# xqtr/PySpecSDR

Measured on AMD Instinct MI355X. Metric: IQ MSamples/sec end-to-end (FFT+dB+FM demod), higher is better.
Workload: dtype complex64 IQ / f64 FFT + dB + post-process + FIR + IIR / dB rows stored as f32 / int16 PCM

## Files before the change

pyspecsdr_amd/csrc/pss_api.cpp:

```cpp
#include <hip/hip_runtime.h>

#include <cstdlib>
#include <cstring>
#include <string>
#include <vector>

#include "pss_ctx.h"

static std::string g_create_err;

int pss_fail(pss_ctx *ctx, int code, const std::string &msg)
{
    if (ctx) ctx->err = msg;
    else g_create_err = msg;
    return code;
}

int pss_hip_check(pss_ctx *ctx, hipError_t e, const char *what)
{
    if (e == hipSuccess) return PSS_OK;
    return pss_fail(ctx, PSS_E_HIP, std::string(what) + ": " + hipGetErrorString(e));
}

int pss_ensure_buffer(pss_ctx *ctx, void **buf, size_t *cap, size_t bytes, const char *what)
{
    if (bytes <= *cap) return PSS_OK;
    if (*buf) {
        hipStreamSynchronize(ctx->stream);
        if (ctx->stream2) hipStreamSynchronize(ctx->stream2);
        hipFree(*buf);
        *buf = nullptr;
        *cap = 0;
    }
    hipError_t e = hipMalloc(buf, bytes);
    if (e != hipSuccess) return pss_fail(ctx, PSS_E_NOMEM, std::string(what) + " hipMalloc: " + hipGetErrorString(e));
    *cap = bytes;
    return PSS_OK;
}

int pss_ensure_scratch(pss_ctx *ctx, size_t bytes)
{
    return pss_ensure_buffer(ctx, &ctx->scratch, &ctx->scratch_bytes, bytes, "scratch");
}

void pss_time_begin(pss_ctx *ctx)
{
    if (ctx->timing && ctx->tdepth++ == 0 && ctx->tfilter.empty()) hipEventRecord(ctx->ev0, ctx->stream);
}
void pss_kernel_begin(pss_ctx *ctx, const char *name)
{
    if (!ctx->timing) return;
    ctx->kskip = !ctx->tfilter.empty() && ctx->tfilter != name;
    if (ctx->kskip) return;
    if (ctx->kused == (int)ctx->krecs.size()) {
        pss_ctx::KRec r{name, nullptr, nullptr};
        hipEventCreate(&r.e0);
        hipEventCreate(&r.e1);
        ctx->krecs.push_back(r);
    }
    ctx->krecs[ctx->kused].name = name;
    hipEventRecord(ctx->krecs[ctx->kused].e0, PSS_STREAM(ctx));
}
void pss_kernel_end(pss_ctx *ctx)
{
    if (!ctx->timing || ctx->kskip) return;
    hipEventRecord(ctx->krecs[ctx->kused].e1, PSS_STREAM(ctx));
    ctx->kused++;
}
void pss_time_end(pss_ctx *ctx)
{
    if (ctx->timing && --ctx->tdepth == 0) {
        if (ctx->tfilter.empty()) hipEventRecord(ctx->ev1, ctx->stream);
        ctx->last_ms = 0.0f;
    }
}

extern "C" int pss_device_count(void)
{
    int n = 0;
    if (hipGetDeviceCount(&n) != hipSuccess) return 0;
    return n;
}

extern "C" int pss_create(int device, pss_ctx **out)
{
    if (!out) return PSS_E_ARG;
    *out = nullptr;
    int n = 0;
    hipError_t e = hipGetDeviceCount(&n);
    if (e != hipSuccess || n <= 0)
        return pss_fail(nullptr, PSS_E_HIP, std::string("no HIP device available (libpss has no CPU fallback): ") +
                                                (e != hipSuccess ? hipGetErrorString(e) : "device count is 0"));
    if (device < 0 || device >= n) return pss_fail(nullptr, PSS_E_ARG, "device index out of range");
    int prev = -1;
    hipGetDevice(&prev);
    e = hipSetDevice(device);
    if (e != hipSuccess) return pss_fail(nullptr, PSS_E_HIP, std::string("hipSetDevice: ") + hipGetErrorString(e));
    struct Restore {
        int prev, dev;
        ~Restore() { if (prev >= 0 && prev != dev) hipSetDevice(prev); }
    } restore{prev, device};
    pss_ctx *ctx = new pss_ctx();
    ctx->device = device;
    { int cus = 0; if (hipDeviceGetAttribute(&cus, hipDeviceAttributeMultiprocessorCount, device) == hipSuccess) ctx->n_cus = cus; }
    { const char *e = getenv("PSS_NO_FUSED"); ctx->no_fused = e && e[0] == '1'; }
    e = hipStreamCreateWithFlags(&ctx->stream, hipStreamNonBlocking);
    if (e == hipSuccess) ctx->own_stream = true;
    if (e == hipSuccess) e = hipEventCreate(&ctx->ev0);
    if (e == hipSuccess) e = hipEventCreate(&ctx->ev1);
    if (e == hipSuccess) e = hipStreamCreateWithFlags(&ctx->stream2, hipStreamNonBlocking);
    if (e == hipSuccess) e = hipEventCreateWithFlags(&ctx->ev_fork, hipEventDisableTiming);
    if (e == hipSuccess) e = hipEventCreateWithFlags(&ctx->ev_join, hipEventDisableTiming);
    if (e != hipSuccess) {
        const std::string msg = std::string("context stream / event creation: ") + hipGetErrorString(e);
        if (ctx->ev0) hipEventDestroy(ctx->ev0);
        if (ctx->ev1) hipEventDestroy(ctx->ev1);
        if (ctx->ev_fork) hipEventDestroy(ctx->ev_fork);
        if (ctx->ev_join) hipEventDestroy(ctx->ev_join);
        if (ctx->stream2) hipStreamDestroy(ctx->stream2);
        if (ctx->own_stream) hipStreamDestroy(ctx->stream);
        delete ctx;
        return pss_fail(nullptr, PSS_E_HIP, msg);
    }
    *out = ctx;
    return PSS_OK;
}

extern "C" void pss_destroy(pss_ctx *ctx)
{
    if (!ctx) return;
    PssDevGuard guard(ctx->device);
    hipStreamSynchronize(ctx->stream);
    if (ctx->comm) pss_comm_free(ctx);
    for (auto &kv : ctx->tw) hipFree(kv.second);
    for (auto &kv : ctx->tw_pf) hipFree(kv.second);
    for (auto &kv : ctx->win) hipFree(kv.second);
    for (auto &kv : ctx->bs) { hipFree(kv.second.d_chirp); hipFree(kv.second.d_B); hipFree(kv.second.d_win); }
    for (auto &kv : ctx->plans) {
        hipFree(kv.second.d_leaf_off); hipFree(kv.second.d_leaf_len); hipFree(kv.second.d_node_l);
        hipFree(kv.second.d_node_r); hipFree(kv.second.d_level_start); hipFree(kv.second.d_roots);
    }
    for (auto &kv : ctx->nfm) if (kv.second.d_rev) hipFree(kv.second.d_rev);
    if (ctx->scratch) hipFree(ctx->scratch);
    if (ctx->scratch_fft) hipFree(ctx->scratch_fft);
    if (ctx->scratch_hil) hipFree(ctx->scratch_hil);
    if (ctx->scratch_iqc) hipFree(ctx->scratch_iqc);
    if (ctx->d_hann) hipFree(ctx->d_hann);
    if (ctx->d_hann_short) hipFree(ctx->d_hann_short);
    if (ctx->st_up) hipStreamDestroy(ctx->st_up);
    if (ctx->st_dn) hipStreamDestroy(ctx->st_dn);
    for (auto &e : ctx->st_ev) if (e) hipEventDestroy(e);
    for (auto &b : ctx->st_buf) if (b) hipFree(b);
    if (ctx->scratch_scan) hipFree(ctx->scratch_scan);
    if (ctx->scratch_pk) hipFree(ctx->scratch_pk);
    if (ctx->scratch_win) hipFree(ctx->scratch_win);
    if (ctx->scratch_db64) hipFree(ctx->scratch_db64);
    if (ctx->scratch_post) hipFree(ctx->scratch_post);
    if (ctx->prog) hipFree(ctx->prog);
    if (ctx->stage) hipFree(ctx->stage);
    for (auto &b : ctx->sq_buf) if (b) hipFree(b);
    if (ctx->sq_pin) hipHostFree(ctx->sq_pin);
    hipEventDestroy(ctx->ev0);
    hipEventDestroy(ctx->ev1);
    hipStreamSynchronize(ctx->stream2);
    hipStreamDestroy(ctx->stream2);
    hipEventDestroy(ctx->ev_fork);
    hipEventDestroy(ctx->ev_join);
    if (ctx->ev_in) hipEventDestroy(ctx->ev_in);
    if (ctx->ev_out) hipEventDestroy(ctx->ev_out);
    for (auto &k : ctx->krecs) { hipEventDestroy(k.e0); hipEventDestroy(k.e1); }
    if (ctx->own_stream) hipStreamDestroy(ctx->stream);
    delete ctx;
}

extern "C" int pss_set_stream(pss_ctx *ctx, void *hip_stream)
{
    if (!ctx) return PSS_E_ARG;
    PSS_GUARD(ctx);
    hipStreamSynchronize(ctx->stream);
    if (ctx->own_stream) hipStreamDestroy(ctx->stream);
    ctx->stream = reinterpret_cast<hipStream_t>(hip_stream);
    ctx->own_stream = false;
    return PSS_OK;
}

extern "C" int pss_order_after(pss_ctx *ctx, void *hip_stream)
{
    if (!ctx) return PSS_E_ARG;
    PSS_GUARD(ctx);
    hipStream_t s = reinterpret_cast<hipStream_t>(hip_stream);
    if (s == ctx->stream) return PSS_OK;
    if (!ctx->ev_in) PSS_HIP(ctx, hipEventCreateWithFlags(&ctx->ev_in, hipEventDisableTiming));
    PSS_HIP(ctx, hipEventRecord(ctx->ev_in, s));
    PSS_HIP(ctx, hipStreamWaitEvent(ctx->stream, ctx->ev_in, 0));
    return PSS_OK;
}

extern "C" int pss_order_before(pss_ctx *ctx, void *hip_stream)
{
    if (!ctx) return PSS_E_ARG;
    PSS_GUARD(ctx);
    hipStream_t s = reinterpret_cast<hipStream_t>(hip_stream);
    if (s == ctx->stream) return PSS_OK;
    if (!ctx->ev_out) PSS_HIP(ctx, hipEventCreateWithFlags(&ctx->ev_out, hipEventDisableTiming));
    PSS_HIP(ctx, hipEventRecord(ctx->ev_out, ctx->stream));
    PSS_HIP(ctx, hipStreamWaitEvent(s, ctx->ev_out, 0));
    return PSS_OK;
}

extern "C" void *pss_get_stream(pss_ctx *ctx) { return ctx ? reinterpret_cast<void *>(ctx->stream) : nullptr; }

extern "C" int pss_set_option(pss_ctx *ctx, const char *key, int value)
{
    if (!ctx || !key) return PSS_E_ARG;
    if (!strcmp(key, "nfm_fused")) { ctx->no_fused = (value == 0); return PSS_OK; }
    if (!strcmp(key, "wfm_fused")) { ctx->no_wfm_fused = (value == 0); return PSS_OK; }
    if (!strcmp(key, "small_batch")) { ctx->no_small_batch = (value == 0); return PSS_OK; }
    if (!strcmp(key, "small_batch_max")) { ctx->small_batch_max = value; return PSS_OK; }
    if (!strcmp(key, "wfm_small_batch_max")) { ctx->wfm_small_batch_max = value; return PSS_OK; }
    if (!strcmp(key, "fuse_post")) { ctx->fuse_post = value != 0; return PSS_OK; }
    if (!strcmp(key, "ssb_rfft")) { ctx->ssb_rfft = value != 0; return PSS_OK; }
    if (!strcmp(key, "ssb_hilbert")) { ctx->ssb_hilbert = value != 0; return PSS_OK; }
    if (!strcmp(key, "hilbert_exact")) { ctx->hilbert_exact = value != 0; return PSS_OK; }
    if (!strcmp(key, "scan_exact")) { ctx->scan_exact = value != 0; return PSS_OK; }
    if (!strcmp(key, "db_exact")) { ctx->db_exact = value != 0; return PSS_OK; }
    if (!strcmp(key, "f64_plain")) { ctx->f64_plain = value != 0; return PSS_OK; }
    if (!strcmp(key, "wfm_corr_copy")) { ctx->wfm_corr_copy = value != 0; return PSS_OK; }
    return pss_fail(ctx, PSS_E_ARG, std::string("unknown option: ") + key);
}

extern "C" int pss_sync(pss_ctx *ctx)
{
    if (!ctx) return PSS_E_ARG;
    PSS_GUARD(ctx);
    return pss_hip_check(ctx, hipStreamSynchronize(ctx->stream), "hipStreamSynchronize");
}

extern "C" const char *pss_last_error(pss_ctx *ctx) { return ctx ? ctx->err.c_str() : g_create_err.c_str(); }

extern "C" int pss_enable_timing(pss_ctx *ctx, int on)
{
    if (!ctx) return PSS_E_ARG;
    PSS_GUARD(ctx);
    ctx->timing = on != 0;
    ctx->tdepth = 0;
    ctx->kused = 0;
    ctx->last_ms = -1.0f;
    return PSS_OK;
}

extern "C" int pss_timing_filter(pss_ctx *ctx, const char *kernel)
{
    if (!ctx) return PSS_E_ARG;
    PSS_GUARD(ctx);
    ctx->tfilter = kernel ? kernel : "";
    ctx->kused = 0;
    ctx->last_ms = -1.0f;
    return PSS_OK;
}

extern "C" float pss_last_kernel_ms(pss_ctx *ctx)
{
    if (!ctx || !ctx->timing || ctx->last_ms < 0.0f || !ctx->tfilter.empty()) return -1.0f;
    PSS_GUARD(ctx);
    if (hipEventSynchronize(ctx->ev1) != hipSuccess) return -1.0f;
    float ms = -1.0f;
    if (hipEventElapsedTime(&ms, ctx->ev0, ctx->ev1) != hipSuccess) return -1.0f;
    return ms;
}

extern "C" int pss_kernel_times(pss_ctx *ctx, char *buf, int buf_len)
{
    if (!ctx || !buf || buf_len < 1) return PSS_E_ARG;
    PSS_GUARD(ctx);
    std::string out;
    if (ctx->timing && ctx->last_ms >= 0.0f) {
        if (ctx->tfilter.empty()) hipEventSynchronize(ctx->ev1);
        else hipStreamSynchronize(ctx->stream);
        for (int i = 0; i < ctx->kused; i++) {
            float ms = 0.0f;
            if (hipEventElapsedTime(&ms, ctx->krecs[i].e0, ctx->krecs[i].e1) != hipSuccess) continue;
            out += ctx->krecs[i].name;
            out += "=" + std::to_string(ms) + ";";
        }
    }
    ctx->kused = 0;
    if ((int)out.size() + 1 > buf_len) return pss_fail(ctx, PSS_E_ARG, "buffer too small");
    memcpy(buf, out.c_str(), out.size() + 1);
    return PSS_OK;
}

namespace {
size_t up256(size_t x) { return (x + 255) & ~(size_t)255; }
}

extern "C" int pss_h_compute_fft(pss_ctx *ctx, const float *h_iq, int n, double *h_db)
{
    if (!ctx) return PSS_E_ARG;
    PSS_GUARD(ctx);
    if (!h_iq || !h_db || n < 1) return pss_fail(ctx, PSS_E_ARG, "bad arguments");
    const size_t o_db = up256(sizeof(float) * 2 * n);
    int r = pss_ensure_buffer(ctx, &ctx->stage, &ctx->stage_bytes, o_db + up256(sizeof(float) * n), "staging");
    if (r) return r;
    char *base = reinterpret_cast<char *>(ctx->stage);
    PSS_HIP(ctx, hipMemcpyAsync(base, h_iq, sizeof(float) * 2 * n, hipMemcpyHostToDevice, ctx->stream));
    r = pss_spectrum_db(ctx, reinterpret_cast<const float *>(base), 1, n, reinterpret_cast<float *>(base + o_db));
    if (r) return r;
    std::vector<float> tmp(n);
    PSS_HIP(ctx, hipMemcpyAsync(tmp.data(), base + o_db, sizeof(float) * n, hipMemcpyDeviceToHost, ctx->stream));
    PSS_HIP(ctx, hipStreamSynchronize(ctx->stream));
    for (int i = 0; i < n; i++) h_db[i] = (double)tmp[i];
// ... 523 lines not shown
```

pyspecsdr_amd/csrc/pss_ctx.h:

```cpp
#pragma once
#include <hip/hip_runtime.h>

#include <array>
#include <functional>
#include <map>
#include <string>
#include <vector>

#include "../../include/pss.h"

struct PssNfmFilt {
    double taps[65];
    double sos[24];
    double zi[8];
    double *d_rev = nullptr;
};

struct PssWfmFilt {
    double lp[18], pilot[30], lmr[30];
    double alpha;
};

struct PssPairwisePlan {
    int n_leaves = 0, n_nodes = 0, n_levels = 0, n_roots = 0;
    int wave_tree = 0;
    int *d_leaf_off = nullptr, *d_leaf_len = nullptr, *d_node_l = nullptr, *d_node_r = nullptr, *d_level_start = nullptr;
    int *d_roots = nullptr;
};

struct pss_ctx {
    int device = 0;
    hipStream_t stream = nullptr;
    bool own_stream = false;
    hipStream_t stream2 = nullptr;
    hipStream_t cur = nullptr;
    hipEvent_t ev_fork = nullptr, ev_join = nullptr;
    hipEvent_t ev_in = nullptr, ev_out = nullptr;
    int n_cus = 0;
    bool iq_c128 = false;
    int fuse_post = 1;
    double target_rate = 22050.0;
    bool wfm_correct = false;
    const float *wfm_scal = nullptr;
    bool wfm_corr_copy = false;
    float *power_out = nullptr;
    bool fork_after_fwd = false;
    bool did_fork = false;
    bool defer_bwd = false;
    std::function<int()> pending_bwd;
    std::string err;
    std::map<int, double2 *> tw;
    std::map<int, double *> win;
    std::map<int, double2 *> tw_pf;
    struct Bluestein { double2 *d_chirp; double2 *d_B; double *d_win; int M; };
    std::map<int, Bluestein> bs;
    std::map<double, PssNfmFilt> nfm;
    std::map<double, std::array<double, 65>> ssb;
    std::map<double, PssWfmFilt> wfm;
    std::map<int, PssPairwisePlan> plans;
    void *scratch = nullptr;
    size_t scratch_bytes = 0;
    void *scratch_iqc = nullptr;
    void *scratch_scan = nullptr;
    size_t scratch_scan_bytes = 0;
    void *scratch_pk = nullptr;
    size_t scratch_pk_bytes = 0;
    void *prog = nullptr;
    unsigned prog_epoch = 0;
    void *scratch_post = nullptr;
    size_t scratch_post_bytes = 0;
    void *scratch_db64 = nullptr;
    size_t scratch_db64_bytes = 0;
    void *scratch_win = nullptr;
    size_t scratch_win_bytes = 0;
    float *d_hann = nullptr;
    float hann_sum = 0.0f;
    hipStream_t st_up = nullptr, st_dn = nullptr;
    hipEvent_t st_ev[6] = {nullptr, nullptr, nullptr, nullptr, nullptr, nullptr};
    void *st_buf[18] = {};
    size_t st_cap[18] = {};
    float *d_hann_short = nullptr;
    float hann_short_sum = 0.0f;
    int hann_short_n = 0;
    size_t scratch_iqc_bytes = 0;
    void *scratch_fft = nullptr;
    size_t scratch_fft_bytes = 0;
    void *scratch_hil = nullptr;
    size_t scratch_hil_bytes = 0;
    void *stage = nullptr;
    size_t stage_bytes = 0;
    bool no_wfm_fused = false;
    long small_batch_max = 8192;
    long wfm_small_batch_max = 6000;
    bool hilbert_exact = false;
    bool ssb_rfft = true;
    bool ssb_hilbert = true;
    bool db_exact = false;
    bool f64_plain = false;
    bool scan_exact = true;
    bool no_small_batch = false;
    bool no_fused = false;
    void *comm = nullptr;
    int comm_rank = 0, comm_n = 1;
    void *sq_buf[3] = {};
    size_t sq_cap[3] = {};
    void *sq_pin = nullptr;
    bool timing = false;
    std::string tfilter;
    bool kskip = false;
    int tdepth = 0;
    hipEvent_t ev0 = nullptr, ev1 = nullptr;
    float last_ms = -1.0f;
    struct KRec { const char *name; hipEvent_t e0, e1; };
    std::vector<KRec> krecs;
    int kused = 0;
};

struct PssDevGuard {
    int prev = -1;
    bool switched = false;
    explicit PssDevGuard(int dev)
    {
        if (hipGetDevice(&prev) == hipSuccess && prev != dev) switched = hipSetDevice(dev) == hipSuccess;
    }
    ~PssDevGuard()
    {
        if (switched) hipSetDevice(prev);
    }
    PssDevGuard(const PssDevGuard &) = delete;
    PssDevGuard &operator=(const PssDevGuard &) = delete;
};
#define PSS_GUARD(ctx) PssDevGuard _pss_dev_guard((ctx)->device)

template <class T>
struct PssScoped {
    T &ref;
    T keep;
    PssScoped(T &r, T v) : ref(r), keep(r) { r = v; }
    ~PssScoped() { ref = keep; }
    PssScoped(const PssScoped &) = delete;
    PssScoped &operator=(const PssScoped &) = delete;
};
using PssFlagScope = PssScoped<bool>;
using PssStreamScope = PssScoped<hipStream_t>;

int pss_fail(pss_ctx *ctx, int code, const std::string &msg);
int pss_hip_check(pss_ctx *ctx, hipError_t e, const char *what);
int pss_ensure_scratch(pss_ctx *ctx, size_t bytes);
int pss_ensure_buffer(pss_ctx *ctx, void **buf, size_t *cap, size_t bytes, const char *what);
void pss_time_begin(pss_ctx *ctx);
void pss_time_end(pss_ctx *ctx);
void pss_kernel_begin(pss_ctx *ctx, const char *name);
void pss_kernel_end(pss_ctx *ctx);

#define PSS_STREAM(ctx) ((ctx)->cur ? (ctx)->cur : (ctx)->stream)

#define PSS_HIP(ctx, call)                                         \
    do {                                                           \
        int _r = pss_hip_check((ctx), (call), #call);              \
        if (_r) return _r;                                         \
    } while (0)

bool pss_hilbert_supported(int n);
int pss_hilbert_rows(pss_ctx *ctx, const double *d_x, long n_rows, int n, double *d_out, int out_mode, unsigned long long *d_maxbits,
                     int16_t *d_pcm);
int pss_fft_tables(pss_ctx *ctx, int n, const double2 **tw, const double **win);
bool pss_post_sel_serves(int n_fft, bool f64);
bool pss_spec_post_serves(const pss_ctx *ctx, int n_fft);
int pss_spec_post_chain(pss_ctx *ctx, const float *d_iq, long n_frames, int n_fft, float *d_db32, double *d_db64, double *d_lo, double *d_hi, int n_halo,
                        int window, int display, int disp_h, int disp_w, int8_t *d_a, int8_t *d_b, double *d_vals);
int pss_chain_vals_f32(pss_ctx *ctx, const float *d_db, long n_frames, int n_fft, float *d_lo, float *d_hi, int n_halo, int window, int display,
                       int disp_h, int disp_w, int8_t *d_a, int8_t *d_b, double *d_vals);
int pss_chain_vals_f64(pss_ctx *ctx, const double *d_db, long n_frames, int n_fft, double *d_lo, double *d_hi, int n_halo, int window, int display,
                       int disp_h, int disp_w, int8_t *d_a, int8_t *d_b, double *d_vals);
bool pss_ssb_fused_supported(int n);
double pss_np_tan(double x);
double pss_np_exp(double x);
int pss_ssb_hilbert_fused(pss_ctx *ctx, const float *d_iq, long n_rows, int n, const double *taps65, double *d_audio, int16_t *d_pcm);
```

pyspecsdr_amd/csrc/pss_fft.hip:

```cpp
#include <hip/hip_runtime.h>

#include <cmath>
#include <vector>

#include "pss_ctx.h"
#include "pss_fft_r16.h"
#include "pss_fft_xl.h"
#include "pss_post.h"
#include "pss_bars.h"
#include "pss_spec_post.h"
#include "pss_hilbert.h"
#include "pss_hilbert_pf.h"

namespace {

constexpr int TPB = 256;

inline int spec_flags(const pss_ctx *ctx) { return (ctx->scan_exact ? pss_r16::FLAG_SCAN_EXACT : 0) | (ctx->db_exact ? pss_r16::FLAG_DB_EXACT : 0); }
constexpr int LOG_NSUB_MAX = 12;
constexpr int STAGE_MAX_N = 16384;
constexpr int PT = 1024;

__device__ __forceinline__ double2 cmul(double2 a, double2 b)
{
// ... 1601 lines not shown
    if (r) { pss_time_end(ctx); return r; }
    double *wlo = reinterpret_cast<double *>(ctx->scratch_win), *whi = wlo + n_frames;
    pss_kernel_begin(ctx, "k_slide_extremes");
    hipLaunchKernelGGL(pss_post::k_slide_extremes<T>, dim3((unsigned)((n_frames + 255) / 256 < 4096 ? (n_frames + 255) / 256 : 4096)),
                       dim3(256), 0, PSS_STREAM(ctx), d_lo, d_hi, n_frames, n_halo, window, wlo, whi);
    pss_kernel_end(ctx);
    const long cells = n_frames * disp_w;
    pss_kernel_begin(ctx, "k_disp_rows");
    const dim3 dgrid((unsigned)((cells + 255) / 256 < 16384 ? (cells + 255) / 256 : 16384));
    if (d_thr)
        hipLaunchKernelGGL((pss_post::k_disp_rows<T, MODE, true>), dgrid, dim3(256), 0, PSS_STREAM(ctx), d_post, wlo, whi, n_frames, len,
                           disp_w, disp_h, d_a, d_b, d_thr);
    else
        hipLaunchKernelGGL((pss_post::k_disp_rows<T, MODE>), dgrid, dim3(256), 0, PSS_STREAM(ctx), d_post, wlo, whi, n_frames, len, disp_w,
                           disp_h, d_a, d_b, (const T *)nullptr);
    pss_kernel_end(ctx);
    pss_time_end(ctx);
    return pss_hip_check(ctx, hipGetLastError(), "k_disp_rows launch");
}

}

extern "C" int pss_spectrum_db_post(pss_ctx *ctx, const float *d_iq, long n_frames, int n_fft, float *d_db, float *d_post,
                                    float *d_row_lo, float *d_row_hi)
{
    if (!ctx) return PSS_E_ARG;
    PSS_GUARD(ctx);
    if (n_frames < 0 || (n_frames > 0 && (!d_iq || !d_db || !d_post))) return pss_fail(ctx, PSS_E_ARG, "pss_spectrum_db_post: null buffer");
    if ((d_row_lo == nullptr) != (d_row_hi == nullptr)) return pss_fail(ctx, PSS_E_ARG, "row extremes: pass both arrays or neither");
    if (n_frames == 0) return PSS_OK;
    int r = pss_spectrum_db(ctx, d_iq, n_frames, n_fft, d_db);
    if (!r) r = spectrum_post(ctx, d_db, n_frames, n_fft, d_post, d_row_lo, d_row_hi);
    return r;
}

extern "C" int pss_spectrum_post(pss_ctx *ctx, const float *d_db, long n_frames, int n_fft, float *d_post)
{
    if (!ctx) return PSS_E_ARG;
    PSS_GUARD(ctx);
    return spectrum_post(ctx, d_db, n_frames, n_fft, d_post, nullptr, nullptr);
}

extern "C" int pss_spectrum_post_extremes(pss_ctx *ctx, const float *d_db, long n_frames, int n_fft, float *d_post, float *d_row_lo,
                                          float *d_row_hi)
{
    if (!ctx) return PSS_E_ARG;
    PSS_GUARD(ctx);
    if (n_frames > 0 && (!d_row_lo || !d_row_hi)) return pss_fail(ctx, PSS_E_ARG, "null row-extremes array");
    return spectrum_post(ctx, d_db, n_frames, n_fft, d_post, d_row_lo, d_row_hi);
}

extern "C" int pss_row_extremes(pss_ctx *ctx, const float *d_rows, long n_rows, int len, float *d_row_lo, float *d_row_hi)
{
    if (!ctx) return PSS_E_ARG;
    PSS_GUARD(ctx);
    return row_extremes<float>(ctx, d_rows, n_rows, len, d_row_lo, d_row_hi);
}
extern "C" int pss_row_extremes_f64(pss_ctx *ctx, const double *d_rows, long n_rows, int len, double *d_row_lo, double *d_row_hi)
{
    if (!ctx) return PSS_E_ARG;
    PSS_GUARD(ctx);
    return row_extremes<double>(ctx, d_rows, n_rows, len, d_row_lo, d_row_hi);
}

extern "C" int pss_spectrum_post_f64(pss_ctx *ctx, const double *d_db, long n_frames, int n_fft, double *d_post, double *d_row_lo, double *d_row_hi)
{
    if (!ctx) return PSS_E_ARG;
    PSS_GUARD(ctx);
    if (n_frames < 0 || n_fft < 5 || (n_frames > 0 && (!d_db || !d_post))) return pss_fail(ctx, PSS_E_ARG, "pss_spectrum_post_f64: bad argument");
    if ((d_row_lo == nullptr) != (d_row_hi == nullptr)) return pss_fail(ctx, PSS_E_ARG, "pss_spectrum_post_f64: row_lo and row_hi go together");
    if (n_frames == 0) return PSS_OK;
    if (!ctx->f64_plain && n_fft >= 8 && post_sel_serves(n_fft, true)) {
        pss_time_begin(ctx);
        const int rq = post_sel_any<double>(ctx, d_db, n_frames, n_fft, d_post, d_row_lo, d_row_hi, nullptr, nullptr, 0);
        pss_time_end(ctx);
        return rq;
    }
    pss_time_begin(ctx);
    pss_kernel_begin(ctx, "k_post_f64");
    hipLaunchKernelGGL(k_post_f64, dim3((unsigned)(n_frames < 2048 ? n_frames : 2048)), dim3(256), 0, PSS_STREAM(ctx), d_db, d_post, n_fft, n_frames);
    pss_kernel_end(ctx);
    int r = pss_hip_check(ctx, hipGetLastError(), "k_post_f64 launch");
    if (!r && d_row_lo) r = row_extremes<double>(ctx, d_post, n_frames, n_fft - 4, d_row_lo, d_row_hi);
    pss_time_end(ctx);
    return r;
}

extern "C" int pss_spectrum_post_thresholds(pss_ctx *ctx, const float *d_db, long n_frames, int n_fft, float *d_row_thr, float *d_row_lo,
                                            float *d_row_hi)
{
    if (!ctx) return PSS_E_ARG;
    PSS_GUARD(ctx);
    if (n_frames > 0 && (!d_row_thr || !d_row_lo || !d_row_hi)) return pss_fail(ctx, PSS_E_ARG, "pss_spectrum_post_thresholds: null buffer");
    return spectrum_post(ctx, d_db, n_frames, n_fft, nullptr, d_row_lo, d_row_hi, d_row_thr);
}
extern "C" int pss_waterfall_rows_db(pss_ctx *ctx, const float *d_db, long n_frames, int n_fft, const float *d_row_thr, const float *d_row_lo,
                                     const float *d_row_hi, int n_halo, int window, int disp_w, int8_t *d_glyph, int8_t *d_colour)
{
    if (!ctx) return PSS_E_ARG;
    PSS_GUARD(ctx);
    if (n_frames > 0 && !d_row_thr) return pss_fail(ctx, PSS_E_ARG, "pss_waterfall_rows_db: null thresholds");
    return display_rows<float, 0>(ctx, d_db, n_frames, n_fft - 4, d_row_lo, d_row_hi, n_halo, window, 1, disp_w, d_glyph, d_colour, d_row_thr);
}
extern "C" int pss_persistence_rows_db(pss_ctx *ctx, const float *d_db, long n_frames, int n_fft, const float *d_row_thr,
                                       const float *d_row_lo, const float *d_row_hi, int n_halo, int window, int disp_h, int disp_w, int8_t *d_y)
{
    if (!ctx) return PSS_E_ARG;
    PSS_GUARD(ctx);
    if (n_frames > 0 && !d_row_thr) return pss_fail(ctx, PSS_E_ARG, "pss_persistence_rows_db: null thresholds");
    return display_rows<float, 1>(ctx, d_db, n_frames, n_fft - 4, d_row_lo, d_row_hi, n_halo, window, disp_h, disp_w, d_y, nullptr, d_row_thr);
}

bool pss_post_sel_serves(int n_fft, bool f64) { return n_fft >= 8 && post_sel_serves(n_fft, f64); }
template <class TR>
static int chain_vals(pss_ctx *ctx, const TR *d_db, long n_frames, int n_fft, TR *d_lo, TR *d_hi, int n_halo, int window, int display, int disp_h,
                      int disp_w, int8_t *d_a, int8_t *d_b, double *d_vals)
{
    if (n_frames == 0) return PSS_OK;
    pss_time_begin(ctx);
    int r = post_sel_any<TR>(ctx, d_db, n_frames, n_fft, (TR *)nullptr, d_lo + n_halo, d_hi + n_halo, (TR *)nullptr, d_vals, disp_w);
    if (!r) r = display == 2 ? display_rows<TR, 2>(ctx, (const TR *)nullptr, n_frames, n_fft - 4, d_lo, d_hi, n_halo, window, 1, disp_w, d_a, d_b, (const TR *)nullptr, d_vals)
              : display ? display_rows<TR, 1>(ctx, (const TR *)nullptr, n_frames, n_fft - 4, d_lo, d_hi, n_halo, window, disp_h, disp_w, d_a, nullptr, (const TR *)nullptr, d_vals)
                        : display_rows<TR, 0>(ctx, (const TR *)nullptr, n_frames, n_fft - 4, d_lo, d_hi, n_halo, window, 1, disp_w, d_a, d_b, (const TR *)nullptr, d_vals);
    pss_time_end(ctx);
    return r;
}
int pss_chain_vals_f32(pss_ctx *ctx, const float *d_db, long n_frames, int n_fft, float *d_lo, float *d_hi, int n_halo, int window, int display,
                       int disp_h, int disp_w, int8_t *d_a, int8_t *d_b, double *d_vals)
{
    return chain_vals<float>(ctx, d_db, n_frames, n_fft, d_lo, d_hi, n_halo, window, display, disp_h, disp_w, d_a, d_b, d_vals);
}
int pss_chain_vals_f64(pss_ctx *ctx, const double *d_db, long n_frames, int n_fft, double *d_lo, double *d_hi, int n_halo, int window, int display,
                       int disp_h, int disp_w, int8_t *d_a, int8_t *d_b, double *d_vals)
{
    return chain_vals<double>(ctx, d_db, n_frames, n_fft, d_lo, d_hi, n_halo, window, display, disp_h, disp_w, d_a, d_b, d_vals);
}

bool pss_spec_post_serves(const pss_ctx *ctx, int n_fft) { return n_fft == 1024 && !ctx->f64_plain; }
int pss_spec_post_chain(pss_ctx *ctx, const float *d_iq, long n_frames, int n_fft, float *d_db32, double *d_db64, double *d_lo, double *d_hi,
                        int n_halo, int window, int display, int disp_h, int disp_w, int8_t *d_a, int8_t *d_b, double *d_vals)
{
    if (!pss_spec_post_serves(ctx, n_fft) || (!d_db32 && !d_db64)) return pss_fail(ctx, PSS_E_ARG, "fused transform + post-process: 1024-point frames, a row buffer");
    if (n_frames == 0) return PSS_OK;
    const double2 *tw;
    const double *win;
    int r = pss_fft_tables(ctx, n_fft, &tw, &win);
    if (r) return r;
    using C = pss_r16::Cfg<2>;
    auto kern = d_db32 ? (d_db64 ? pss_sp::k_spectrum_post<true, true> : pss_sp::k_spectrum_post<true, false>) : pss_sp::k_spectrum_post<false, true>;
    const size_t lds = (size_t)C::FPW * C::EX * sizeof(double2) + (size_t)C::TW2 * sizeof(double2);
    const long cap = 256L * 2 * 2;
    if (lds > 64 * 1024) PSS_HIP(ctx, hipFuncSetAttribute(reinterpret_cast<const void *>(kern), hipFuncAttributeMaxDynamicSharedMemorySize, (int)lds));
    const long groups = (n_frames + C::FPW - 1) / C::FPW;
    pss_time_begin(ctx);
    pss_kernel_begin(ctx, "k_spectrum_post");
    hipLaunchKernelGGL(kern, dim3((unsigned)(groups < cap ? groups : cap)), dim3(256), lds, PSS_STREAM(ctx), reinterpret_cast<const float2 *>(d_iq), d_db32,
                       d_db64, tw, win, n_frames, d_lo + n_halo, d_hi + n_halo, d_vals, disp_w);
    pss_kernel_end(ctx);
    r = pss_hip_check(ctx, hipGetLastError(), "k_spectrum_post launch");
    if (!r) r = display == 2 ? display_rows<double, 2>(ctx, (const double *)nullptr, n_frames, n_fft - 4, d_lo, d_hi, n_halo, window, 1, disp_w, d_a, d_b, (const double *)nullptr, d_vals)
              : display ? display_rows<double, 1>(ctx, (const double *)nullptr, n_frames, n_fft - 4, d_lo, d_hi, n_halo, window, disp_h, disp_w, d_a, nullptr, (const double *)nullptr, d_vals)
                        : display_rows<double, 0>(ctx, (const double *)nullptr, n_frames, n_fft - 4, d_lo, d_hi, n_halo, window, 1, disp_w, d_a, d_b, (const double *)nullptr, d_vals);
    pss_time_end(ctx);
    return r;
}

extern "C" int pss_waterfall_rows(pss_ctx *ctx, const float *d_post, long n_frames, int len, const float *d_row_lo,
                                  const float *d_row_hi, int n_halo, int window, int disp_w, int8_t *d_glyph, int8_t *d_colour)
{
    if (!ctx) return PSS_E_ARG;
    PSS_GUARD(ctx);
    return display_rows<float, 0>(ctx, d_post, n_frames, len, d_row_lo, d_row_hi, n_halo, window, 1, disp_w, d_glyph, d_colour);
}
extern "C" int pss_waterfall_rows_f64(pss_ctx *ctx, const double *d_post, long n_frames, int len, const double *d_row_lo,
                                      const double *d_row_hi, int n_halo, int window, int disp_w, int8_t *d_glyph, int8_t *d_colour)
{
    if (!ctx) return PSS_E_ARG;
    PSS_GUARD(ctx);
    return display_rows<double, 0>(ctx, d_post, n_frames, len, d_row_lo, d_row_hi, n_halo, window, 1, disp_w, d_glyph, d_colour);
}
extern "C" int pss_gradient_rows(pss_ctx *ctx, const float *d_post, long n_frames, int len, const float *d_row_lo,
                                 const float *d_row_hi, int n_halo, int window, int disp_w, int8_t *d_glyph, int8_t *d_colour)
{
    if (!ctx) return PSS_E_ARG;
    PSS_GUARD(ctx);
    return display_rows<float, 2>(ctx, d_post, n_frames, len, d_row_lo, d_row_hi, n_halo, window, 1, disp_w, d_glyph, d_colour);
}
extern "C" int pss_gradient_rows_f64(pss_ctx *ctx, const double *d_post, long n_frames, int len, const double *d_row_lo,
                                     const double *d_row_hi, int n_halo, int window, int disp_w, int8_t *d_glyph, int8_t *d_colour)
{
    if (!ctx) return PSS_E_ARG;
    PSS_GUARD(ctx);
    return display_rows<double, 2>(ctx, d_post, n_frames, len, d_row_lo, d_row_hi, n_halo, window, 1, disp_w, d_glyph, d_colour);
}
extern "C" int pss_persistence_rows(pss_ctx *ctx, const float *d_post, long n_frames, int len, const float *d_row_lo,
                                    const float *d_row_hi, int n_halo, int window, int disp_h, int disp_w, int8_t *d_y)
{
    if (!ctx) return PSS_E_ARG;
    PSS_GUARD(ctx);
    return display_rows<float, 1>(ctx, d_post, n_frames, len, d_row_lo, d_row_hi, n_halo, window, disp_h, disp_w, d_y, nullptr);
}
extern "C" int pss_persistence_rows_f64(pss_ctx *ctx, const double *d_post, long n_frames, int len, const double *d_row_lo,
                                        const double *d_row_hi, int n_halo, int window, int disp_h, int disp_w, int8_t *d_y)
{
    if (!ctx) return PSS_E_ARG;
    PSS_GUARD(ctx);
    return display_rows<double, 1>(ctx, d_post, n_frames, len, d_row_lo, d_row_hi, n_halo, window, disp_h, disp_w, d_y, nullptr);
}

extern "C" int pss_waterfall_cells(pss_ctx *ctx, const float *d_rows, int n_rows, int len, int disp_h, int disp_w,
                                   int8_t *d_glyph, int8_t *d_colour)
{
    if (!ctx) return PSS_E_ARG;
    PSS_GUARD(ctx);
    if (!d_rows || !d_glyph || !d_colour || n_rows < 1 || len < 2 || disp_h < 1 || disp_w < 1)
        return pss_fail(ctx, PSS_E_ARG, "bad waterfall arguments");
    pss_kernel_begin(ctx, "k_cells");
    hipLaunchKernelGGL((k_cells<float, 0>), dim3(1), dim3(1024), 0, PSS_STREAM(ctx), d_rows, n_rows, len, disp_h, disp_w,
                       d_glyph, d_colour, 0, n_rows);
    pss_kernel_end(ctx);
    return pss_hip_check(ctx, hipGetLastError(), "k_cells launch");
}

extern "C" int pss_persistence_cells(pss_ctx *ctx, const float *d_rows, int n_rows, int len, int disp_h, int disp_w,
                                     int8_t *d_colour)
{
    if (!ctx) return PSS_E_ARG;
    PSS_GUARD(ctx);
    if (!d_rows || !d_colour || n_rows < 1 || len < 2 || disp_h < 1 || disp_w < 1)
        return pss_fail(ctx, PSS_E_ARG, "bad persistence arguments");
    pss_kernel_begin(ctx, "k_cells");
    hipLaunchKernelGGL((k_cells<float, 1>), dim3(1), dim3(1024), 0, PSS_STREAM(ctx), d_rows, n_rows, len, disp_h, disp_w,
                       (int8_t *)nullptr, d_colour, 0, n_rows);
    pss_kernel_end(ctx);
    return pss_hip_check(ctx, hipGetLastError(), "k_cells launch");
}

template <class T>
static int launch_spectrogram(pss_ctx *ctx, const T *d_rows, long n_rows, int len, int disp_h, int disp_w, int8_t *d_glyph,
                              int8_t *d_colour, double *d_range)
{
    if (!ctx) return PSS_E_ARG;
    PSS_GUARD(ctx);
    if (!d_rows || !d_glyph || !d_colour || n_rows < 0 || len < 2 || disp_h < 1 || disp_w < 1)
        return pss_fail(ctx, PSS_E_ARG, "bad spectrogram arguments");
    if (n_rows == 0) return PSS_OK;
    pss_kernel_begin(ctx, "k_spectrogram");
    hipLaunchKernelGGL(k_spectrogram<T>, dim3((unsigned)(n_rows < 4096 ? n_rows : 4096)), dim3(len <= 4096 ? 256 : 1024), 0,
                       PSS_STREAM(ctx), d_rows, n_rows, len, disp_h, disp_w, d_glyph, d_colour, d_range);
    pss_kernel_end(ctx);
    return pss_hip_check(ctx, hipGetLastError(), "k_spectrogram launch");
}

extern "C" int pss_spectrogram_cells(pss_ctx *ctx, const float *d_rows, long n_rows, int len, int disp_h, int disp_w,
                                     int8_t *d_glyph, int8_t *d_colour, double *d_range)
{
    return launch_spectrogram<float>(ctx, d_rows, n_rows, len, disp_h, disp_w, d_glyph, d_colour, d_range);
}

extern "C" int pss_spectrogram_cells_f64(pss_ctx *ctx, const double *d_rows, long n_rows, int len, int disp_h, int disp_w,
                                         int8_t *d_glyph, int8_t *d_colour, double *d_range)
{
    return launch_spectrogram<double>(ctx, d_rows, n_rows, len, disp_h, disp_w, d_glyph, d_colour, d_range);
}

namespace {
constexpr int BARS_REG_MAX_LEN = 4092;

template <class T, int EPL, int W>
int launch_bars_reg(pss_ctx *ctx, const T *d_rows, long n_rows, int len, int disp_h, int disp_w, int8_t *d_height, int8_t *d_level, double *d_range)
{
    constexpr int RPW = W == 1 ? 4 : 1;
    const size_t lds = (size_t)RPW * 64 * W * EPL * sizeof(double);
    auto kern = k_spectrum_bars<T, EPL, W>;
    if (lds + 512 > 64 * 1024)
        PSS_HIP(ctx, hipFuncSetAttribute(reinterpret_cast<const void *>(kern), hipFuncAttributeMaxDynamicSharedMemorySize, (int)lds));
    long per_cu = (long)((160 * 1024) / (lds + 512));
    per_cu = per_cu < 1 ? 1 : (per_cu > 6 ? 6 : per_cu);
    const long groups = (n_rows + RPW - 1) / RPW, cap = 256L * per_cu;
    pss_kernel_begin(ctx, "k_spectrum_bars");
    hipLaunchKernelGGL(kern, dim3((unsigned)(groups < cap ? groups : cap)), dim3(W == 1 ? 256 : 64 * W), lds, PSS_STREAM(ctx), d_rows, n_rows, len, disp_h,
                       disp_w, d_height, d_level, d_range);
    pss_kernel_end(ctx);
    return PSS_OK;
}

template <class T>
int spectrum_bars(pss_ctx *ctx, const T *d_rows, long n_rows, int len, int disp_h, int disp_w, int8_t *d_height, int8_t *d_level, double *d_range)
{
    if (n_rows < 0 || len < 1 || disp_h < 1 || disp_h > 127 || disp_w < 1 || (n_rows > 0 && (!d_rows || !d_height || !d_level)))
        return pss_fail(ctx, PSS_E_ARG, "pss_spectrum_bars: bad argument (len >= 1, 1 <= disp_h <= 127, disp_w >= 1, non-null buffers)");
    if (n_rows == 0) return PSS_OK;
    pss_time_begin(ctx);
    int r = PSS_OK;
    if (len <= 256) r = launch_bars_reg<T, 4, 1>(ctx, d_rows, n_rows, len, disp_h, disp_w, d_height, d_level, d_range);
    else if (len <= 1024) r = launch_bars_reg<T, 16, 1>(ctx, d_rows, n_rows, len, disp_h, disp_w, d_height, d_level, d_range);
    else if (len <= 2048) r = launch_bars_reg<T, 32, 1>(ctx, d_rows, n_rows, len, disp_h, disp_w, d_height, d_level, d_range);
    else if (len <= BARS_REG_MAX_LEN) r = launch_bars_reg<T, 16, 4>(ctx, d_rows, n_rows, len, disp_h, disp_w, d_height, d_level, d_range);
    else {
        pss_kernel_begin(ctx, "k_spectrum_bars");
        hipLaunchKernelGGL((k_spectrogram<T, true>), dim3((unsigned)(n_rows < 4096 ? n_rows : 4096)), dim3(1024), 0, PSS_STREAM(ctx), d_rows, n_rows, len,
                           disp_h, disp_w, d_height, d_level, d_range);
        pss_kernel_end(ctx);
    }
    pss_time_end(ctx);
    return r ? r : pss_hip_check(ctx, hipGetLastError(), "k_spectrum_bars launch");
}

bool bars_cells_args_ok(const int8_t *height, const int8_t *level, long n_rows, int disp_h, int disp_w, const int8_t *glyph, const int8_t *colour)
{
    return n_rows >= 0 && disp_h >= 1 && disp_h <= 127 && disp_w >= 1 && (n_rows == 0 || (height && level && glyph && colour));
}
// ... 211 lines not shown
```

pyspecsdr_amd/csrc/pss_spec_post.h:

```cpp
#pragma once

namespace pss_sp {

using namespace pss_r16;

template <bool ROW32, bool ROW64>
__global__ __launch_bounds__(256, 2) void k_spectrum_post(const float2 *__restrict__ iq, float *__restrict__ db32, double *__restrict__ db64,
                                                       const double2 *__restrict__ tw, const double *__restrict__ win, long n_frames,
                                                       double *__restrict__ row_lo, double *__restrict__ row_hi, double *__restrict__ vals,
                                                       int disp_w)
{
    using C = Cfg<2>;
    constexpr int R3 = C::R3, T = C::T, N = C::N, FPW = C::FPW;
    static_assert(T == 64, "a frame is one wavefront");
    constexpr int EPL = 16;
    using PC = pss_post::PostCfg<EPL, double>;
    static_assert((size_t)(T + 1) * PC::S * sizeof(double) <= (size_t)C::EX * sizeof(double2), "the staged row fits the frame's exchange buffer");
    extern __shared__ __align__(16) unsigned char smem[];
    double2 *ex_all = reinterpret_cast<double2 *>(smem);
    double2 *tw2 = ex_all + (size_t)FPW * C::EX;
    const int tid = threadIdx.x;
    const int fl = __builtin_amdgcn_readfirstlane(tid / T);
    const int t = tid % T;
    double2 *ex = ex_all + (size_t)fl * C::EX;
    double *stage = reinterpret_cast<double *>(ex);
    double2 tw1[16];
    double w[16];
    tw1[0] = make_double2(1.0, 0.0);
#pragma unroll
    for (int k2 = 1; k2 < 16; k2++) tw1[k2] = tw[(size_t)t * k2];
#pragma unroll
    for (int n2 = 0; n2 < 16; n2++) w[n2] = win[t + T * n2];
    if (tid < R3 * 16) {
        const int m1 = tid / 16, j2 = tid % 16;
        tw2[C::tw2_slot(tid)] = tw[(size_t)(m1 * j2) * 16];
    }
    __syncthreads();
    const long groups = (n_frames + FPW - 1) / FPW;
    float2 nx[16];
    auto fetch = [&](long g) {
        const long f = g * FPW + fl;
        const float2 *x = iq + (size_t)(f < n_frames ? f : 0) * N;
#pragma unroll
        for (int n2 = 0; n2 < 16; n2++) nx[n2] = x[t + T * n2];
    };
    if ((long)blockIdx.x < groups) fetch(blockIdx.x);
    int phase = 0;
    for (long g = blockIdx.x; g < groups; g += gridDim.x) {
        const long f = g * FPW + fl;
        const bool valid = f < n_frames;
        double2 v[16];
#pragma unroll
        for (int n2 = 0; n2 < 16; n2++) v[n2] = make_double2((double)nx[n2].x * w[n2], (double)nx[n2].y * w[n2]);
        if (g + gridDim.x < groups) fetch(g + gridDim.x);
        const long f_first = g * FPW;
        const long rows_here = n_frames - f_first < FPW ? n_frames - f_first : FPW;
        const __amdgpu_buffer_rsrc_t ro32 = make_rsrc((ROW32 && db32) ? db32 + (size_t)f_first * N : nullptr, (ROW32 && db32) ? (unsigned)(rows_here * N * 4) : 0u);
        const __amdgpu_buffer_rsrc_t ro64 = make_rsrc((ROW64 && db64) ? db64 + (size_t)f_first * N : nullptr, (ROW64 && db64) ? (unsigned)(rows_here * N * 8) : 0u);
        const int lane_el = fl * N + t;
        double dbv[16];
        auto emit = [&](int i, int k, double2 X) {
            const double d64 = db64_of_exact(power_of(X));
            const int e0 = ((k - t) + N / 2) & (N - 1);
            if constexpr (ROW64) buf_store_f64(ro64, lane_el * 8, e0 * 8, d64);
            if constexpr (ROW32) buf_store_f32(ro32, lane_el * 4, e0 * 4, (float)d64);
            dbv[i] = d64;
        };
        r16_core<2, true>(v, ex, tw1, tw2, t, emit);
        frame_sync<true>();
#pragma unroll
        for (int i = 0; i < 16; i++) {
            const int c = i / R3, j1 = i % R3;
            const int e = (((256 * j1 + T * c) + N / 2) & (N - 1)) + t;
            stage[(e / EPL) * PC::S + (e % EPL)] = dbv[i];
        }
        frame_sync<true>();
        if (valid) {
            int slot[PC::Q];
#pragma unroll
            for (int j = 0; j < PC::Q; j++) slot[j] = 0;
            pss_post::post_row_staged<EPL, 1, true, double>(stage, slot, t, N - 4, nullptr, fl, t, phase, nullptr, row_lo, row_hi, f, nullptr, vals, disp_w);
        }
        frame_sync<true>();
    }
}

}
```

Before: 70240.

## Replace grid-stride frame loop with atomic-ticket dynamic scheduling in spectrum post kernel

The spectrum+post kernel now hands out frame groups dynamically through a global atomic ticket counter instead of a fixed grid-stride walk. Each block claims its next group one iteration ahead so it can keep prefetching, and it stops after a per-block quota. The grid is resized from the number of groups and that quota. Two ticket counters alternate between launches so each launch can zero the other one, which avoids a memset per call. The goal is better load balance and a shorter tail across CUs, at the cost of one atomic per iteration and a full block barrier in place of the per-frame sync.

Result: no change. 70780 (median of 6 runs) (+0.8%).

```diff
diff --git a/pyspecsdr_amd/csrc/pss_api.cpp b/pyspecsdr_amd/csrc/pss_api.cpp
--- a/pyspecsdr_amd/csrc/pss_api.cpp
+++ b/pyspecsdr_amd/csrc/pss_api.cpp
@@ -157,6 +157,7 @@
     if (ctx->scratch_db64) hipFree(ctx->scratch_db64);
     if (ctx->scratch_post) hipFree(ctx->scratch_post);
     if (ctx->prog) hipFree(ctx->prog);
+    if (ctx->post_tickets) hipFree(ctx->post_tickets);
     if (ctx->stage) hipFree(ctx->stage);
     for (auto &b : ctx->sq_buf) if (b) hipFree(b);
     if (ctx->sq_pin) hipHostFree(ctx->sq_pin);
diff --git a/pyspecsdr_amd/csrc/pss_ctx.h b/pyspecsdr_amd/csrc/pss_ctx.h
--- a/pyspecsdr_amd/csrc/pss_ctx.h
+++ b/pyspecsdr_amd/csrc/pss_ctx.h
@@ -67,6 +67,8 @@
     size_t scratch_pk_bytes = 0;
     void *prog = nullptr;
     unsigned prog_epoch = 0;
+    void *post_tickets = nullptr;
+    unsigned post_seq = 0;
     void *scratch_post = nullptr;
     size_t scratch_post_bytes = 0;
     void *scratch_db64 = nullptr;
diff --git a/pyspecsdr_amd/csrc/pss_fft.hip b/pyspecsdr_amd/csrc/pss_fft.hip
--- a/pyspecsdr_amd/csrc/pss_fft.hip
+++ b/pyspecsdr_amd/csrc/pss_fft.hip
@@ -1777,12 +1777,21 @@
     const long cap = 256L * 2 * 2;
     if (lds > 64 * 1024) PSS_HIP(ctx, hipFuncSetAttribute(reinterpret_cast<const void *>(kern), hipFuncAttributeMaxDynamicSharedMemorySize, (int)lds));
     const long groups = (n_frames + C::FPW - 1) / C::FPW;
+    const long need = (groups + pss_sp::SPEC_POST_QUOTA - 1) / pss_sp::SPEC_POST_QUOTA;
+    const long grid = groups < cap ? groups : (need + need / 2 > cap ? need + need / 2 : cap);
+    if (!ctx->post_tickets) {
+        PSS_HIP(ctx, hipMalloc(&ctx->post_tickets, 2 * 128));
+        PSS_HIP(ctx, hipMemsetAsync(ctx->post_tickets, 0, 2 * 128, PSS_STREAM(ctx)));
+    }
+    unsigned *tk_now = reinterpret_cast<unsigned *>(ctx->post_tickets) + 32 * (ctx->post_seq & 1u);
+    unsigned *tk_next = reinterpret_cast<unsigned *>(ctx->post_tickets) + 32 * (~ctx->post_seq & 1u);
     pss_time_begin(ctx);
     pss_kernel_begin(ctx, "k_spectrum_post");
-    hipLaunchKernelGGL(kern, dim3((unsigned)(groups < cap ? groups : cap)), dim3(256), lds, PSS_STREAM(ctx), reinterpret_cast<const float2 *>(d_iq), d_db32,
-                       d_db64, tw, win, n_frames, d_lo + n_halo, d_hi + n_halo, d_vals, disp_w);
+    hipLaunchKernelGGL(kern, dim3((unsigned)grid), dim3(256), lds, PSS_STREAM(ctx), reinterpret_cast<const float2 *>(d_iq), d_db32,
+                       d_db64, tw, win, n_frames, d_lo + n_halo, d_hi + n_halo, d_vals, disp_w, tk_now, tk_next);
     pss_kernel_end(ctx);
     r = pss_hip_check(ctx, hipGetLastError(), "k_spectrum_post launch");
+    if (!r) ctx->post_seq++;
     if (!r) r = display == 2 ? display_rows<double, 2>(ctx, (const double *)nullptr, n_frames, n_fft - 4, d_lo, d_hi, n_halo, window, 1, disp_w, d_a, d_b, (const double *)nullptr, d_vals)
               : display ? display_rows<double, 1>(ctx, (const double *)nullptr, n_frames, n_fft - 4, d_lo, d_hi, n_halo, window, disp_h, disp_w, d_a, nullptr, (const double *)nullptr, d_vals)
                         : display_rows<double, 0>(ctx, (const double *)nullptr, n_frames, n_fft - 4, d_lo, d_hi, n_halo, window, 1, disp_w, d_a, d_b, (const double *)nullptr, d_vals);
diff --git a/pyspecsdr_amd/csrc/pss_spec_post.h b/pyspecsdr_amd/csrc/pss_spec_post.h
--- a/pyspecsdr_amd/csrc/pss_spec_post.h
+++ b/pyspecsdr_amd/csrc/pss_spec_post.h
@@ -4,11 +4,13 @@
 
 using namespace pss_r16;
 
+constexpr int SPEC_POST_QUOTA = 16;
+
 template <bool ROW32, bool ROW64>
 __global__ __launch_bounds__(256, 2) void k_spectrum_post(const float2 *__restrict__ iq, float *__restrict__ db32, double *__restrict__ db64,
                                                        const double2 *__restrict__ tw, const double *__restrict__ win, long n_frames,
                                                        double *__restrict__ row_lo, double *__restrict__ row_hi, double *__restrict__ vals,
-                                                       int disp_w)
+                                                       int disp_w, unsigned *__restrict__ ticket, unsigned *__restrict__ ticket_next)
 {
     using C = Cfg<2>;
     constexpr int R3 = C::R3, T = C::T, N = C::N, FPW = C::FPW;
@@ -19,7 +21,11 @@
     extern __shared__ __align__(16) unsigned char smem[];
     double2 *ex_all = reinterpret_cast<double2 *>(smem);
     double2 *tw2 = ex_all + (size_t)FPW * C::EX;
+    __shared__ unsigned claimed[2];
     const int tid = threadIdx.x;
+    if (tid == 0 && blockIdx.x == 0) __hip_atomic_store(ticket_next, 0u, __ATOMIC_RELAXED, __HIP_MEMORY_SCOPE_AGENT);
+    unsigned tk = 0;
+    if (tid == 0) tk = __hip_atomic_fetch_add(ticket, 1u, __ATOMIC_RELAXED, __HIP_MEMORY_SCOPE_AGENT);
     const int fl = __builtin_amdgcn_readfirstlane(tid / T);
     const int t = tid % T;
     double2 *ex = ex_all + (size_t)fl * C::EX;
@@ -35,6 +41,7 @@
         const int m1 = tid / 16, j2 = tid % 16;
         tw2[C::tw2_slot(tid)] = tw[(size_t)(m1 * j2) * 16];
     }
+    if (tid == 0) claimed[0] = tk;
     __syncthreads();
     const long groups = (n_frames + FPW - 1) / FPW;
     float2 nx[16];
@@ -44,15 +51,18 @@
 #pragma unroll
         for (int n2 = 0; n2 < 16; n2++) nx[n2] = x[t + T * n2];
     };
-    if ((long)blockIdx.x < groups) fetch(blockIdx.x);
+    long g = blockIdx.x;
+    long g_next = (long)gridDim.x + (long)__builtin_amdgcn_readfirstlane(claimed[0]);
+    fetch(g);
     int phase = 0;
-    for (long g = blockIdx.x; g < groups; g += gridDim.x) {
+    for (int it = 0; g < groups; it++) {
+        const bool more = g_next < groups;
         const long f = g * FPW + fl;
         const bool valid = f < n_frames;
         double2 v[16];
 #pragma unroll
         for (int n2 = 0; n2 < 16; n2++) v[n2] = make_double2((double)nx[n2].x * w[n2], (double)nx[n2].y * w[n2]);
-        if (g + gridDim.x < groups) fetch(g + gridDim.x);
+        if (more) fetch(g_next);
         const long f_first = g * FPW;
         const long rows_here = n_frames - f_first < FPW ? n_frames - f_first : FPW;
         const __amdgpu_buffer_rsrc_t ro32 = make_rsrc((ROW32 && db32) ? db32 + (size_t)f_first * N : nullptr, (ROW32 && db32) ? (unsigned)(rows_here * N * 4) : 0u);
@@ -67,6 +77,9 @@
             dbv[i] = d64;
         };
         r16_core<2, true>(v, ex, tw1, tw2, t, emit);
+        const bool draw = more && it + 2 < SPEC_POST_QUOTA;
+        unsigned drawn = 0;
+        if (tid == 0 && draw) drawn = __hip_atomic_fetch_add(ticket, 1u, __ATOMIC_RELAXED, __HIP_MEMORY_SCOPE_AGENT);
         frame_sync<true>();
 #pragma unroll
         for (int i = 0; i < 16; i++) {
@@ -81,7 +94,10 @@
             for (int j = 0; j < PC::Q; j++) slot[j] = 0;
             pss_post::post_row_staged<EPL, 1, true, double>(stage, slot, t, N - 4, nullptr, fl, t, phase, nullptr, row_lo, row_hi, f, nullptr, vals, disp_w);
         }
-        frame_sync<true>();
+        if (tid == 0) claimed[(it + 1) & 1] = drawn;
+        __syncthreads();
+        g = g_next;
+        g_next = draw ? (long)gridDim.x + (long)__builtin_amdgcn_readfirstlane(claimed[(it + 1) & 1]) : groups;
     }
 }
 
```
